# nnaisense/evotorch

Measured on NVIDIA H100. Metric: PGPE generations/sec at popsize=1Mxdim=10k (Rastrigin, fp32), higher is better.
Workload: dtype f32

## Files before the change

### evotorch_b200/_native.py

```python

from __future__ import annotations

import ctypes
import os
from ctypes import c_float, c_int, c_int64, c_size_t, c_uint64, c_void_p
from typing import Optional

import torch

_PKG = os.path.dirname(os.path.abspath(__file__))
LIB_PATH = os.path.join(_PKG, "lib", "libevok.so")

_P = c_void_p
_SIGNATURES = {
    "evok_abi_version": (c_int, []),
    "evok_launch_count": (c_uint64, []),
    "evok_error_string": (ctypes.c_char_p, [c_int]),
    "evok_sample_eval": (c_int, [c_int, _P, c_int64, _P, _P, c_int64, c_int64, c_int64, c_int, c_uint64, c_uint64, _P, _P, _P]),
    "evok_eval": (c_int, [c_int, _P, c_int64, c_int64, c_int64, _P, _P]),
    "evok_rank_workspace_bytes": (c_size_t, [c_int64]),
    "evok_rank": (c_int, [c_int, _P, c_int64, c_int, _P, _P, _P, c_size_t, _P]),
    "evok_argsort": (c_int, [_P, c_int64, c_int, _P, _P, c_size_t, _P]),
    "evok_sample_batched": (c_int, [_P, c_int64, c_int64, _P, c_int64, _P, c_int64, c_int64, c_int64, c_int64, c_int, c_uint64, c_uint64, _P]),
    "evok_rank_batched": (c_int, [c_int, _P, c_int64, c_int64, c_int, _P, _P, c_size_t, _P]),
# ... 2 lines not shown
    "evok_grad_batched_workspace_bytes": (c_size_t, [c_int64, c_int64, c_int64]),
    "evok_grad_batched": (c_int, [c_int, _P, c_int64, c_int64, _P, _P, c_int64, _P, c_int64, c_int64, c_int64, c_int64, c_float, c_float, _P, _P, _P,
                                  c_size_t, _P]),
    "evok_clipup_batched": (c_int, [_P, c_int64, c_int64, _P, _P, _P, _P, _P, _P]),
    "evok_sigma_update_batched": (c_int, [_P, _P, c_int64, c_int64, _P, c_int, _P, _P, _P, _P]),
    "evok_rank_table": (c_int, [_P, c_int64, c_int, _P, _P, _P, c_size_t, _P]),
    "evok_cholesky_workspace_bytes": (c_size_t, [c_int64]),
    "evok_cholesky": (c_int, [_P, c_int64, c_int64, _P, c_int64, _P, c_size_t, _P]),
    "evok_cmaes_row_weights": (c_int, [_P, _P, c_int64, c_int64, c_int64, c_int, _P, _P, _P]),
    "evok_cmaes_vector_update": (c_int, [_P, _P, c_int64, _P, _P, _P, _P, _P, c_int64, _P, c_int, _P, _P, _P]),
    "evok_sample_eval_sq": (c_int, [c_int, _P, c_int64, _P, _P, c_int64, c_int64, c_int64, c_uint64, c_uint64, _P, _P, _P, _P]),
    "evok_sepcma_workspace_bytes": (c_size_t, [c_int64, c_int64]),
    "evok_sepcma_moments": (c_int, [_P, _P, c_int, c_int64, c_int64, c_int64, c_uint64, c_uint64, _P, _P, _P, _P, _P, c_size_t, _P]),
    "evok_sepcma_update": (c_int, [_P, _P, _P, c_int64, _P, _P, _P, _P, _P, _P, _P, _P, _P, _P, c_int64, _P, c_int, c_int64, c_float, c_float, _P,
                                   _P]),
    "evok_weights_adjust": (c_int, [_P, c_int64, c_int, _P]),
    "evok_elite_mask": (c_int, [_P, c_int64, c_int64, _P, _P, c_size_t, _P]),
    "evok_grad_workspace_bytes": (c_size_t, [c_int64, c_int64]),
    "evok_grad": (c_int, [c_int, _P, c_int64, _P, _P, _P, c_int64, c_int64, c_float, c_float, _P, _P, _P, c_size_t, _P]),
    "evok_grad_regen": (c_int, [c_int, _P, _P, _P, c_int64, c_int64, c_int64, c_uint64, c_uint64, _P, c_float, c_float, _P, _P, _P,
                                c_size_t, _P]),
    "evok_grad_hybrid": (c_int, [c_int, _P, c_int64, _P, _P, _P, c_int64, c_int64, c_int64, c_uint64, c_uint64, _P, c_int, c_float, c_float, _P,
                                 _P, _P, c_size_t, _P]),
    "evok_grad_auto_split": (c_int, [c_int64]),
    "evok_grad_power_limit_mw": (c_int64, [c_int]),
    "evok_clipup_step": (c_int, [_P, c_int64, _P, c_float, c_float, c_float, _P, _P, _P]),
    "evok_adam_step": (c_int, [_P, c_int64, _P, _P, c_int64, c_float, c_float, c_float, c_float, _P, _P, _P]),
    "evok_sgd_step": (c_int, [_P, c_int64, _P, c_int, c_float, c_float, _P, _P, _P]),
    "evok_axpy": (c_int, [_P, c_int64, c_float, _P, _P]),
    "evok_sigma_update": (c_int, [_P, _P, c_int64, c_float, c_int, _P, c_float, _P, c_float, _P, c_float, _P]),
    "evok_cem_finalize": (c_int, [_P, _P, _P, c_int64, c_int64, _P, _P, _P]),
    "evok_mlp_parameter_length": (c_int64, [c_int, _P]),
    "evok_mlp_forward": (c_int, [_P, c_int64, _P, c_int64, _P, c_int64, c_int64, c_int, _P, _P, _P]),
    "evok_mlp_forward_prep": (c_int, [_P, c_int64, _P, c_int64, _P, c_int64, c_int64, c_int, _P, _P, _P, _P, _P, c_float, c_float, c_float, _P, _P,
                                      c_size_t, _P]),
    "evok_mlp_forward_shared_supported": (c_int, [c_int, _P]),
    "evok_mlp_forward_shared_workspace_bytes": (c_size_t, [c_int64, c_int64, c_int, _P]),
    "evok_mlp_forward_shared": (c_int, [_P, c_int64, c_int64, _P, c_int64, c_int64, c_int, _P, _P, _P, _P, c_size_t, _P]),
    "evok_gemm_gather_rows": (c_int, [_P, c_int64, c_int64, c_int64, c_int64, _P, c_int64, c_int64, c_int64, c_int64, c_int, _P, c_int64, _P]),
    "evok_gemm_gather_rows_workspace_bytes": (c_size_t, [c_int64, c_int64]),
    "evok_gemm_gather_rows_ws": (c_int, [_P, c_int64, c_int64, c_int64, c_int64, _P, c_int64, c_int64, c_int64, c_int64, c_int, _P, c_int64, c_int, _P, c_size_t, _P]),
    "evok_gemm_workspace_bytes": (c_size_t, [c_int64, c_int64, c_int64]),
    "evok_gemm_nt": (c_int, [_P, c_int64, _P, c_int64, c_int64, c_int64, c_int64, _P, c_int64, _P, c_int64, _P, _P, _P, c_size_t, _P]),
    "evok_gemm_nt_affine": (c_int, [_P, c_int64, _P, c_int64, c_int64, c_int64, c_int64, _P, c_int64, _P, _P, c_int64, _P, _P, c_size_t, _P]),
    "evok_transpose_pair": (c_int, [_P, c_int64, c_int64, c_int64, _P, _P, _P, c_int64, _P]),
    "evok_transpose_scale": (c_int, [_P, c_int64, c_int64, c_int64, _P, _P, c_int64, _P]),
# ... 102 lines not shown
```

### evotorch_b200/csrc/evok_common.cuh

```cuda
#pragma once

#include <cuda_runtime.h>
#include <stdint.h>

#include "../../include/evok.h"

#define EVOK_CHECK_LAUNCH_N(n)                       \
  do {                                               \
    cudaError_t e__ = cudaPeekAtLastError();         \
    if (e__ != cudaSuccess) return (int)e__;         \
    evok::count_launches(n);                         \
  } while (0)
#define EVOK_CHECK_LAUNCH() EVOK_CHECK_LAUNCH_N(1)

namespace evok {

extern unsigned long long g_launch_count;
inline void count_launches(int n) { __atomic_fetch_add(&g_launch_count, (unsigned long long)n, __ATOMIC_RELAXED); }

constexpr int kWarp = 32;
constexpr int kNumSMs = 132;

struct PeerSink {
  void* data[EVOK_MAX_PEERS];
// ... 78 lines not shown
}

__device__ __forceinline__ void box_muller(uint32_t a, uint32_t b, float& z0, float& z1) {
  const float u1 = fmaf((float)a, 2.3283064365386963e-10f, 1.1641532182693481e-10f);
  const float th = fmaf((float)b, 1.4629180792671596e-09f, 7.314590396335798e-10f);
  const float r = sqrt_approx(lg2_approx(u1) * -1.3862943611198906f);
  float s, c;
  __sincosf(th, &s, &c);
  z0 = r * c;
  z1 = r * s;
}

__device__ __forceinline__ void normals4(const PhiloxKey& key, uint32_t stream_word, uint64_t unit, uint32_t q, float z[4]) {
  U4 c;
  c.x = q;
  c.y = (uint32_t)unit;
  c.z = (uint32_t)(unit >> 32);
  c.w = stream_word;
  const U4 r = philox4x32_10(c, key);
  box_muller(r.x, r.y, z[0], z[1]);
  box_muller(r.z, r.w, z[2], z[3]);
}

__device__ __forceinline__ float warp_sum(float v) {
#pragma unroll
  for (int o = 16; o > 0; o >>= 1) v += __shfl_xor_sync(0xffffffffu, v, o);
  return v;
}
__device__ __forceinline__ double warp_sum(double v) {
#pragma unroll
  for (int o = 16; o > 0; o >>= 1) v += __shfl_xor_sync(0xffffffffu, v, o);
  return v;
}

template <typename T>
__device__ __forceinline__ T block_sum(T v, T* smem ) {
  const int lane = threadIdx.x & 31, wid = threadIdx.x >> 5, nw = (blockDim.x + 31) >> 5;
  v = warp_sum(v);
  __syncthreads();
  if (lane == 0) smem[wid] = v;
  __syncthreads();
  if (wid == 0) {
    T t = lane < nw ? smem[lane] : T(0);
    t = warp_sum(t);
    if (lane == 0) smem[32] = t;
  }
// ... 91 lines not shown
```

### evotorch_b200/csrc/evok_grad.cu

```cuda
#include <dlfcn.h>

#include <atomic>
#include <cstdlib>

#include "evok_common.cuh"

#ifndef EVOK_GRAD_TMA_DEFAULT
#define EVOK_GRAD_TMA_DEFAULT 1
#endif

namespace evok {

#ifndef EVOK_GRAD_UNROLL
#define EVOK_GRAD_UNROLL 4
#endif
#ifndef EVOK_GRAD_MINB
#define EVOK_GRAD_MINB 4
#endif
#ifndef EVOK_GRAD_CTAS_PER_SM
#define EVOK_GRAD_CTAS_PER_SM 4
#endif
constexpr int kGradThreads = 256;
constexpr int kGradUnroll = EVOK_GRAD_UNROLL;
constexpr int kMaxResidentCtas = kNumSMs * 8;
// ... 231 lines not shown
static int launch_finalize(const float* partial, int n_chunks, int64_t D, float scale_mu, float scale_sigma, float* out_mu, float* out_sigma,
                           const GradPush* push, cudaStream_t st) {
  const unsigned grid = (unsigned)((D + 255) / 256);
  if (push) grad_finalize_push_kernel<<<grid, 256, 0, st>>>(partial, n_chunks, D, scale_mu, scale_sigma, push->sink, push->epoch, push->done);
  else grad_finalize_kernel<<<grid, 256, 0, st>>>(partial, n_chunks, D, scale_mu, scale_sigma, out_mu, out_sigma);
  EVOK_CHECK_LAUNCH();
  return 0;
}

#ifndef EVOK_GRAD_TMA_ROWS
#define EVOK_GRAD_TMA_ROWS 4
#endif
#ifndef EVOK_GRAD_TMA_STAGES
#define EVOK_GRAD_TMA_STAGES 4
#endif
#ifndef EVOK_GRAD_TMA_CTAS_PER_SM
#define EVOK_GRAD_TMA_CTAS_PER_SM 3
#endif
constexpr int kTmaRows = EVOK_GRAD_TMA_ROWS;
constexpr int kTmaStages = EVOK_GRAD_TMA_STAGES;
constexpr int kTmaCols = 1024;
constexpr int kTmaConsumers = 256;
constexpr int kTmaThreads = kTmaConsumers + 32;
constexpr size_t kTmaSmemBytes = (size_t)kTmaStages * kTmaRows * kTmaCols * sizeof(float) + 2 * kTmaStages * sizeof(uint64_t) + 128;

__device__ __forceinline__ uint32_t smem_u32(const void* p) { return (uint32_t)__cvta_generic_to_shared(p); }
__device__ __forceinline__ void mbar_init(uint64_t* bar, uint32_t count) {
  asm volatile("mbarrier.init.shared::cta.b64 [%0], %1;" ::"r"(smem_u32(bar)), "r"(count) : "memory");
}
__device__ __forceinline__ void mbar_expect_tx(uint64_t* bar, uint32_t bytes) {
  asm volatile("mbarrier.arrive.expect_tx.shared::cta.b64 _, [%0], %1;" ::"r"(smem_u32(bar)), "r"(bytes) : "memory");
}
__device__ __forceinline__ void mbar_arrive(uint64_t* bar) {
  asm volatile("mbarrier.arrive.shared::cta.b64 _, [%0];" ::"r"(smem_u32(bar)) : "memory");
}
__device__ __forceinline__ void mbar_wait(uint64_t* bar, uint32_t parity) {
  asm volatile(
      "{\n"
      ".reg .pred P1;\n"
      "LAB_WAIT:\n"
      "mbarrier.try_wait.parity.shared::cta.b64 P1, [%0], %1;\n"
      "@P1 bra DONE;\n"
      "bra LAB_WAIT;\n"
      "DONE:\n"
      "}" ::"r"(smem_u32(bar)), "r"(parity) : "memory");
}
__device__ __forceinline__ void bulk_load(void* dst_smem, const void* src_gmem, uint32_t bytes, uint64_t* bar) {
  asm volatile("cp.async.bulk.shared::cluster.global.mbarrier::complete_tx::bytes [%0], [%1], %2, [%3];" ::"r"(smem_u32(dst_smem)),
               "l"(src_gmem), "r"(bytes), "r"(smem_u32(bar))
               : "memory");
}

constexpr int kSplitPeriod = 16;
__device__ __forceinline__ uint32_t rebuilt_mask(int split) {
  uint32_t m = 0;
#pragma unroll
  for (int k = 0; k < kSplitPeriod; ++k)
    if ((k + 1) * split / kSplitPeriod > k * split / kSplitPeriod) m |= 1u << k;
  return m;
}
__device__ __forceinline__ bool group_rebuilt(uint32_t mask, int64_t g) { return (mask >> ((int)g & (kSplitPeriod - 1))) & 1u; }

template <bool SYM>
__global__ void __launch_bounds__(kTmaThreads, EVOK_GRAD_TMA_CTAS_PER_SM)
    grad_partial_tma_kernel(int form, const float* __restrict__ X, int64_t ldx, const float* __restrict__ w, const float* __restrict__ mu,
                            const float* __restrict__ sigma, int64_t n_units, int64_t D, int64_t units_per_chunk, int split, uint64_t unit0,
                            const __grid_constant__ PhiloxKey key, const uint32_t* __restrict__ stream_off, float* __restrict__ partial) {
  extern __shared__ __align__(128) unsigned char smem_raw[];
  float* tiles = reinterpret_cast<float*>(smem_raw);
  uint64_t* full = reinterpret_cast<uint64_t*>(smem_raw + (size_t)kTmaStages * kTmaRows * kTmaCols * sizeof(float));
  uint64_t* empty = full + kTmaStages;

  const int tid = threadIdx.x, warp = tid >> 5, lane = tid & 31;
  const int64_t col0 = (int64_t)blockIdx.x * kTmaCols;
  const int64_t width = min((int64_t)kTmaCols, D - col0);
  const int64_t r_begin = (int64_t)blockIdx.y * units_per_chunk;
  const int64_t r_end = min(n_units, r_begin + units_per_chunk);
  const int64_t n_rows = r_end - r_begin;
  const int64_t n_groups = (n_rows + kTmaRows - 1) / kTmaRows;
  const int64_t row_stride = (SYM ? 2 : 1) * ldx;
  const uint32_t mask = rebuilt_mask(split);

  if (tid == 0) {
    for (int s = 0; s < kTmaStages; ++s) {
      mbar_init(&full[s], 1);
      mbar_init(&empty[s], kTmaConsumers / 32);
    }
    asm volatile("fence.mbarrier_init.release.cluster;" ::: "memory");
  }
  __syncthreads();

  if (warp == kTmaConsumers / 32) {
    if (lane == 0) {
      const uint32_t row_bytes = (uint32_t)(width * sizeof(float));
      int64_t t = 0;
      for (int64_t g = 0; g < n_groups; ++g) {
        if (group_rebuilt(mask, g)) continue;
        const int s = (int)(t % kTmaStages);
        const uint32_t use = (uint32_t)(t / kTmaStages);
        ++t;
        if (use > 0) mbar_wait(&empty[s], (use - 1) & 1);
        const int64_t r0 = r_begin + g * kTmaRows;
        const int rows = (int)min((int64_t)kTmaRows, r_end - r0);
        mbar_expect_tx(&full[s], rows * row_bytes);
        float* dst = tiles + (size_t)s * kTmaRows * kTmaCols;
        for (int i = 0; i < rows; ++i) bulk_load(dst + (size_t)i * kTmaCols, X + (r0 + i) * row_stride + col0, row_bytes, &full[s]);
      }
    }
    return;
  }

  const int64_t col = col0 + (int64_t)tid * 4;
  const bool active = col < D;
  const uint32_t sw = key.stream_lo + (stream_off ? __ldg(stream_off) : 0u);
  const int frm = SYM ? EVOK_GRAD_SYMMETRIC : form;
  float m[4], sg[4], c1[4], c0[4];
#pragma unroll
  for (int c = 0; c < 4; ++c) {
    sg[c] = active ? __ldg(sigma + col + c) : 1.0f;
    m[c] = active ? __ldg(mu + col + c) : 0.0f;
    if (frm == EVOK_GRAD_EXP) {
      c1[c] = __fdiv_rn(1.0f, sg[c] * sg[c]);
      c0[c] = 1.0f;
    } else if (frm == EVOK_GRAD_MOMENTS) {
      c1[c] = 1.0f;
      c0[c] = 0.0f;
    } else {
      c1[c] = __fdiv_rn(1.0f, sg[c]);
      c0[c] = sg[c];
    }
  }
  float s1[4] = {0.f, 0.f, 0.f, 0.f}, s2[4] = {0.f, 0.f, 0.f, 0.f};

  int64_t t = 0;
  for (int64_t g = 0; g < n_groups; ++g) {
    const int64_t r0 = r_begin + g * kTmaRows;
    const int rows = (int)min((int64_t)kTmaRows, r_end - r0);
    float a[kTmaRows], b[kTmaRows];
    bool need[kTmaRows];
#pragma unroll
    for (int i = 0; i < kTmaRows; ++i) {
      a[i] = b[i] = 0.0f;
      if (i < rows) {
        if (SYM) {
          const float wp = __ldg(w + 2 * (r0 + i)), wm = __ldg(w + 2 * (r0 + i) + 1);
          a[i] = 0.5f * (wp - wm);
          b[i] = 0.5f * (wp + wm);
        } else {
          a[i] = b[i] = __ldg(w + r0 + i);
        }
      }
      need[i] = a[i] != 0.0f || b[i] != 0.0f;
    }
    if (group_rebuilt(mask, g)) {
      if (active) {
        float x[kTmaRows][4];
#pragma unroll
        for (int i = 0; i < kTmaRows; ++i) {
          float z[4];
          normals4(key, sw, unit0 + (uint64_t)(r0 + i), (uint32_t)(col >> 2), z);
#pragma unroll
          for (int c = 0; c < 4; ++c) x[i][c] = fmaf(sg[c], z[c], m[c]);
        }
#pragma unroll
        for (int i = 0; i < kTmaRows; ++i) {
          if (need[i]) {
#pragma unroll
            for (int c = 0; c < 4; ++c) {
              const float e = x[i][c] - m[c];
              s1[c] = fmaf(a[i], e, s1[c]);
              s2[c] = fmaf(b[i], fmaf(e * e, c1[c], -c0[c]), s2[c]);
            }
          }
        }
      }
      continue;
    }
    const int s = (int)(t % kTmaStages);
    const uint32_t use = (uint32_t)(t / kTmaStages);
    ++t;
    mbar_wait(&full[s], use & 1);
    const float4* tile = reinterpret_cast<const float4*>(tiles + (size_t)s * kTmaRows * kTmaCols) + tid;
    if (active) {
      float4 v4[kTmaRows];
#pragma unroll
      for (int i = 0; i < kTmaRows; ++i) v4[i] = tile[(size_t)i * (kTmaCols / 4)];
#pragma unroll
      for (int i = 0; i < kTmaRows; ++i) {
        if (need[i]) {
          const float4 v = v4[i];
          const float x[4] = {v.x, v.y, v.z, v.w};
#pragma unroll
          for (int c = 0; c < 4; ++c) {
            const float e = x[c] - m[c];
            s1[c] = fmaf(a[i], e, s1[c]);
            s2[c] = fmaf(b[i], fmaf(e * e, c1[c], -c0[c]), s2[c]);
          }
        }
      }
    }
    __syncwarp();
    if (lane == 0) mbar_arrive(&empty[s]);
  }
  if (active) {
    float* p1 = partial + ((int64_t)blockIdx.y * 2 + 0) * D + col;
    float* p2 = partial + ((int64_t)blockIdx.y * 2 + 1) * D + col;
#pragma unroll
    for (int c = 0; c < 4; ++c) {
      p1[c] = s1[c];
      p2[c] = s2[c];
    }
  }
}

struct GradPlan {
  int vec, tx, n_coltiles, n_chunks;
  int64_t units_per_chunk;
};

static GradPlan plan_grad(int64_t n_units, int64_t D, bool vec_ok) {
  GradPlan p;
  p.vec = vec_ok ? 4 : 1;
  const int64_t col_threads = (D + p.vec - 1) / p.vec;
  p.tx = 32;
  while (p.tx < kGradThreads && p.tx < col_threads) p.tx <<= 1;
  p.n_coltiles = (int)((col_threads + p.tx - 1) / p.tx);
// ... 41 lines not shown
    cudaGetLastError();
    return -1;
  }
  void* nvml = dlopen("libnvidia-ml.so.1", RTLD_NOW | RTLD_LOCAL);
  if (!nvml) return -1;
  using init_t = int (*)();
  using by_bus_t = int (*)(const char*, void**);
  using limit_t = int (*)(void*, unsigned int*);
  const auto init = reinterpret_cast<init_t>(dlsym(nvml, "nvmlInit_v2"));
  const auto shutdown = reinterpret_cast<init_t>(dlsym(nvml, "nvmlShutdown"));
  const auto by_bus = reinterpret_cast<by_bus_t>(dlsym(nvml, "nvmlDeviceGetHandleByPciBusId_v2"));
  const auto limit = reinterpret_cast<limit_t>(dlsym(nvml, "nvmlDeviceGetEnforcedPowerLimit"));
  int64_t mw = -1;
  if (init && shutdown && by_bus && limit && init() == 0) {
    void* handle = nullptr;
    unsigned int v = 0;
    if (by_bus(bus_id, &handle) == 0 && limit(handle, &v) == 0) mw = v;
    shutdown();
  }
  dlclose(nvml);
  return mw;
}

static int device_auto_split() {
  constexpr int kMaxDevices = 64;
  static std::atomic<int> resolved[kMaxDevices];
  int device = 0;
  if (cudaGetDevice(&device) != cudaSuccess || device < 0 || device >= kMaxDevices) {
    cudaGetLastError();
    return kAutoSplitCapped;
  }
  int s = resolved[device].load(std::memory_order_relaxed);
  if (s == 0) {
    s = auto_split_for_power(enforced_power_limit_mw(device)) + 1;
    resolved[device].store(s, std::memory_order_relaxed);
  }
  return s - 1;
}

static int grad_impl(int form, const float* X, int64_t ldx, const float* w, const float* mu, const float* sigma, int64_t row0, int64_t n_rows,
                     int64_t D, bool regen, uint64_t seed, uint64_t stream_id, const uint32_t* stream_off, float scale_mu, float scale_sigma, float* out_mu,
                     float* out_sigma, void* ws, size_t ws_bytes, void* stream, const GradPush* push = nullptr, int split = 0) {
  if (!w || !mu || !sigma || !ws || (!regen && !X) || (!push && (!out_mu || !out_sigma))) return EVOK_E_NULLPTR;
  if (form < EVOK_GRAD_SEPARABLE || form > EVOK_GRAD_MOMENTS) return EVOK_E_BADENUM;
  if (n_rows < 0 || D <= 0 || row0 < 0 || (!regen && ldx < D) || split < -1 || split > kSplitPeriod) return EVOK_E_BADSIZE;
  const bool sym = form == EVOK_GRAD_SYMMETRIC;
  if (sym && ((n_rows & 1) || (row0 & 1))) return EVOK_E_ODDROWS;
  if (ws_bytes < evok_grad_workspace_bytes(n_rows, D)) return EVOK_E_WORKSPACE;
  cudaStream_t st = (cudaStream_t)stream;
  const int64_t n_units = sym ? n_rows / 2 : n_rows;
  const bool vec_ok = regen ? true : ((D % 4 == 0) && (ldx % 4 == 0) && aligned16(X));
  const uint64_t unit0 = (uint64_t)(sym ? row0 / 2 : row0);
  GradPlan p = plan_grad(n_units, D, vec_ok);
  float* partial = (float*)ws;
  if (n_units == 0 && push) return launch_finalize(partial, 0, D, scale_mu, scale_sigma, nullptr, nullptr, push, st);
  if (n_units == 0) {
    cudaMemsetAsync(out_mu, 0, (size_t)D * 4, st);
    cudaMemsetAsync(out_sigma, 0, (size_t)D * 4, st);
    return 0;
  }
  const char* tma_env = getenv("EVOK_GRAD_TMA");
  const int use_tma = tma_env ? atoi(tma_env) : EVOK_GRAD_TMA_DEFAULT;
  if (use_tma && !regen && vec_ok && form != EVOK_GRAD_MOMENTS && D >= 512 && n_units >= 4096) {
    const int n_coltiles = (int)((D + kTmaCols - 1) / kTmaCols);
    int64_t chunks = (int64_t)kNumSMs * EVOK_GRAD_TMA_CTAS_PER_SM / n_coltiles;
    if (chunks < 1) chunks = 1;
    if (chunks > 65535) chunks = 65535;
    const int64_t upc = (n_units + chunks - 1) / chunks;
    const int n_chunks = (int)((n_units + upc - 1) / upc);
    dim3 grid(n_coltiles, n_chunks);
    const int rebuilt = split < 0 ? device_auto_split() : split;
    const PhiloxKey key = make_philox_key(seed, stream_id);
    auto kernel = sym ? grad_partial_tma_kernel<true> : grad_partial_tma_kernel<false>;
    cudaFuncSetAttribute(kernel, cudaFuncAttributeMaxDynamicSharedMemorySize, (int)kTmaSmemBytes);
    kernel<<<grid, kTmaThreads, kTmaSmemBytes, st>>>(form, X, ldx, w, mu, sigma, n_units, D, upc, rebuilt, unit0, key, stream_off, partial);
    EVOK_CHECK_LAUNCH();
    return launch_finalize(partial, n_chunks, D, scale_mu, scale_sigma, out_mu, out_sigma, push, st);
  }
  if (regen) {
    if (sym) launch_partial<4, true, true>(p, form, X, ldx, w, mu, sigma, n_units, D, unit0, seed, stream_id, stream_off, partial, st);
    else launch_partial<4, false, true>(p, form, X, ldx, w, mu, sigma, n_units, D, unit0, seed, stream_id, stream_off, partial, st);
  } else if (vec_ok) {
    if (sym) launch_partial<4, true, false>(p, form, X, ldx, w, mu, sigma, n_units, D, unit0, seed, stream_id, stream_off, partial, st);
    else launch_partial<4, false, false>(p, form, X, ldx, w, mu, sigma, n_units, D, unit0, seed, stream_id, stream_off, partial, st);
  } else {
    if (sym) launch_partial<1, true, false>(p, form, X, ldx, w, mu, sigma, n_units, D, unit0, seed, stream_id, stream_off, partial, st);
    else launch_partial<1, false, false>(p, form, X, ldx, w, mu, sigma, n_units, D, unit0, seed, stream_id, stream_off, partial, st);
  }
  EVOK_CHECK_LAUNCH();
  return launch_finalize(partial, p.n_chunks, D, scale_mu, scale_sigma, out_mu, out_sigma, push, st);
}

}

using namespace evok;

extern "C" EVOK_API size_t evok_grad_workspace_bytes(int64_t n_rows, int64_t D) {
  (void)n_rows;
  if (D <= 0) return 256;
  return ((size_t)kMaxResidentCtas * 1024 + 2 * (size_t)D + 64) * sizeof(float);
}

extern "C" EVOK_API int evok_grad(int form, const float* X, int64_t ldx, const float* w, const float* mu, const float* sigma, int64_t n_rows,
                         int64_t D, float scale_mu, float scale_sigma, float* out_mu, float* out_sigma, void* ws, size_t ws_bytes,
                         void* stream) {
  return grad_impl(form, X, ldx, w, mu, sigma, 0, n_rows, D, false, 0, 0, nullptr, scale_mu, scale_sigma, out_mu, out_sigma, ws, ws_bytes, stream);
}

extern "C" EVOK_API int evok_grad_regen(int form, const float* w, const float* mu, const float* sigma, int64_t row0, int64_t n_rows, int64_t D,
                               uint64_t seed, uint64_t stream_id, const uint32_t* stream_offset_dev, float scale_mu, float scale_sigma,
                               float* out_mu, float* out_sigma, void* ws, size_t ws_bytes, void* stream) {
  return grad_impl(form, nullptr, 0, w, mu, sigma, row0, n_rows, D, true, seed, stream_id, stream_offset_dev, scale_mu, scale_sigma, out_mu, out_sigma, ws,
                   ws_bytes, stream);
}

extern "C" EVOK_API int evok_grad_hybrid(int form, const float* X, int64_t ldx, const float* w, const float* mu, const float* sigma, int64_t row0,
                                         int64_t n_rows, int64_t D, uint64_t seed, uint64_t stream_id, const uint32_t* stream_offset_dev, int split,
                                         float scale_mu, float scale_sigma, float* out_mu, float* out_sigma, void* ws, size_t ws_bytes, void* stream) {
  return grad_impl(form, X, ldx, w, mu, sigma, row0, n_rows, D, false, seed, stream_id, stream_offset_dev, scale_mu, scale_sigma, out_mu, out_sigma, ws,
                   ws_bytes, stream, nullptr, split);
}

extern "C" EVOK_API int evok_grad_auto_split(int64_t power_limit_mw) { return auto_split_for_power(power_limit_mw); }

extern "C" EVOK_API int64_t evok_grad_power_limit_mw(int device) { return enforced_power_limit_mw(device); }

extern "C" EVOK_API size_t evok_sepcma_workspace_bytes(int64_t n_rows, int64_t D) {
  return evok_grad_workspace_bytes(n_rows, D) + (size_t)kMaxResidentCtas * sizeof(float);
}

extern "C" EVOK_API int evok_sepcma_moments(const float* aw, const float* q, int active, int64_t row0, int64_t n_rows, int64_t D, uint64_t seed,
                                            uint64_t stream_id, const uint32_t* stream_offset_dev, float* local, float* S2, float* wsum, void* ws,
                                            size_t ws_bytes, void* stream) {
  if (!aw || (active && !q) || !local || !S2 || !wsum || !ws) return EVOK_E_NULLPTR;
  if (n_rows <= 0 || D <= 0 || row0 < 0) return EVOK_E_BADSIZE;
  if (ws_bytes < evok_sepcma_workspace_bytes(n_rows, D)) return EVOK_E_WORKSPACE;
  cudaStream_t st = (cudaStream_t)stream;
  const GradPlan p = plan_grad(n_rows, D, true);
  float* partial = (float*)ws;
  const SepWeights sep{q, active, partial + evok_grad_workspace_bytes(n_rows, D) / sizeof(float)};
  launch_partial<4, false, true, true>(p, EVOK_GRAD_MOMENTS, nullptr, 0, aw, nullptr, nullptr, n_rows, D, (uint64_t)row0, seed, stream_id,
                                       stream_offset_dev, partial, st, 1, nullptr, &sep);
  EVOK_CHECK_LAUNCH();
  grad_finalize_kernel<true><<<(unsigned)((D + 255) / 256), 256, 0, st>>>(partial, p.n_chunks, D, 1.0f, 1.0f, local, S2, 0, sep.wsum_partial, wsum);
// ... 77 lines not shown
```

### evotorch_b200/ops.py

```python

from __future__ import annotations

import ctypes
import math
from typing import Optional

import torch

from . import _native as nat
from .tools.readonlytensor import as_plain_tensor

OBJ_NONE, OBJ_SPHERE, OBJ_RASTRIGIN, OBJ_ACKLEY = 0, 1, 2, 3
OBJECTIVE_IDS = {"sphere": OBJ_SPHERE, "rastrigin": OBJ_RASTRIGIN, "ackley": OBJ_ACKLEY}
RANK_IDS = {"centered": 0, "linear": 1, "nes": 2, "normalized": 3, "raw": 4}
GRAD_SEPARABLE, GRAD_SYMMETRIC, GRAD_EXP, GRAD_MOMENTS = 0, 1, 2, 3
NAN = float("nan")


_timers: Optional[dict] = None


def enable_timers() -> None:
    global _timers
    _timers = {}
# ... 317 lines not shown
    with _timed("grad"):
        rc = nat.lib().evok_grad(form, X.data_ptr(), X.stride(0), w.data_ptr(), mu.data_ptr(), sigma.data_ptr(), n, D, scale_mu,
                                 scale_sigma, out_mu.data_ptr(), out_sigma.data_ptr(), ws.data_ptr(), ws.numel(), nat.stream_of(X))
    nat.check(rc, "evok_grad")
    return out_mu, out_sigma


def grad_regen(form: int, w: torch.Tensor, mu: torch.Tensor, sigma: torch.Tensor, *, seed: int, stream_id: int, row0: int,
               scale_mu: float, scale_sigma: float, out_mu: Optional[torch.Tensor] = None,
               out_sigma: Optional[torch.Tensor] = None, stream_offset: Optional[torch.Tensor] = None) -> tuple:
    n, D = w.numel(), mu.numel()
    _vec(w, "weights"); _vec(mu, "mu"); _vec(sigma, "sigma", D)
    out_mu, out_sigma = _out_pair(mu, out_mu, out_sigma)
    ws = nat.workspace(mu.device, nat.lib().evok_grad_workspace_bytes(n, D), "grad")
    with _timed("grad_regen"):
        rc = nat.lib().evok_grad_regen(form, w.data_ptr(), mu.data_ptr(), sigma.data_ptr(), row0, n, D, seed, stream_id,
                                       _offset_ptr(stream_offset), scale_mu, scale_sigma, out_mu.data_ptr(), out_sigma.data_ptr(),
                                       ws.data_ptr(), ws.numel(), nat.stream_of(mu))
    nat.check(rc, "evok_grad_regen")
    return out_mu, out_sigma


GRAD_SPLIT_PERIOD = 16


def grad_hybrid(form: int, X: torch.Tensor, w: torch.Tensor, mu: torch.Tensor, sigma: torch.Tensor, *, seed: int, stream_id: int, row0: int,
                scale_mu: float, scale_sigma: float, split: int = -1, out_mu: Optional[torch.Tensor] = None,
                out_sigma: Optional[torch.Tensor] = None, stream_offset: Optional[torch.Tensor] = None) -> tuple:
    _mat(X, "samples")
    n, D = X.shape
    _vec(w, "weights", n); _vec(mu, "mu", D); _vec(sigma, "sigma", D)
    if not -1 <= split <= GRAD_SPLIT_PERIOD:
        raise ValueError(f"split: expected -1 .. {GRAD_SPLIT_PERIOD}, got {split}")
    out_mu, out_sigma = _out_pair(mu, out_mu, out_sigma)
    ws = nat.workspace(X.device, nat.lib().evok_grad_workspace_bytes(n, D), "grad")
    with _timed("grad_hybrid"):
        rc = nat.lib().evok_grad_hybrid(form, X.data_ptr(), X.stride(0), w.data_ptr(), mu.data_ptr(), sigma.data_ptr(), row0, n, D,
                                        seed, stream_id, _offset_ptr(stream_offset), int(split), scale_mu, scale_sigma,
                                        out_mu.data_ptr(), out_sigma.data_ptr(), ws.data_ptr(), ws.numel(), nat.stream_of(X))
    nat.check(rc, "evok_grad_hybrid")
    return out_mu, out_sigma


def clipup_step(g: torch.Tensor, velocity: torch.Tensor, stepsize: float, momentum: float, max_speed: float,
                step_out: Optional[torch.Tensor] = None, mu: Optional[torch.Tensor] = None) -> None:
    D = g.numel()
    _vec(g, "g"); _vec(velocity, "velocity", D)
    with _timed("mu_step"):
        rc = nat.lib().evok_clipup_step(g.data_ptr(), D, velocity.data_ptr(), stepsize, momentum, max_speed, nat.ptr(step_out),
                                        nat.ptr(mu), nat.stream_of(g))
    nat.check(rc, "evok_clipup_step")


def adam_step(g: torch.Tensor, m: torch.Tensor, v: torch.Tensor, t: int, lr: float, beta1: float, beta2: float, eps: float,
              step_out: Optional[torch.Tensor] = None, mu: Optional[torch.Tensor] = None) -> None:
    D = g.numel()
    _vec(g, "g"); _vec(m, "m", D); _vec(v, "v", D)
    rc = nat.lib().evok_adam_step(g.data_ptr(), D, m.data_ptr(), v.data_ptr(), t, lr, beta1, beta2, eps, nat.ptr(step_out), nat.ptr(mu),
                                  nat.stream_of(g))
    nat.check(rc, "evok_adam_step")


# ... 301 lines not shown
```

### include/evok.h

```cpp
#ifndef EVOK_H_
#define EVOK_H_

#include <stddef.h>
#include <stdint.h>

#ifdef __cplusplus
extern "C" {
#endif

#define EVOK_ABI_VERSION 1

#if defined(__GNUC__)
#define EVOK_API __attribute__((visibility("default")))
#else
#define EVOK_API
#endif

#define EVOK_E_NULLPTR (-1)
#define EVOK_E_BADSIZE (-2)
#define EVOK_E_BADENUM (-3)
#define EVOK_E_WORKSPACE (-4)
#define EVOK_E_ODDROWS (-5)
#define EVOK_E_ALIGN (-6)

#define EVOK_MAX_PEERS 16

#define EVOK_OBJ_NONE 0
#define EVOK_OBJ_SPHERE 1
#define EVOK_OBJ_RASTRIGIN 2
#define EVOK_OBJ_ACKLEY 3
#define EVOK_OBJ_COUNT 4

#define EVOK_RANK_CENTERED 0
#define EVOK_RANK_LINEAR 1
#define EVOK_RANK_NES 2
#define EVOK_RANK_NORMALIZED 3
#define EVOK_RANK_RAW 4

#define EVOK_GRAD_SEPARABLE 0
#define EVOK_GRAD_SYMMETRIC 1
#define EVOK_GRAD_EXP 2
#define EVOK_GRAD_MOMENTS 3

int evok_abi_version(void);
uint64_t evok_launch_count(void);
const char* evok_error_string(int code);

int evok_sample_eval(int objective, float* X, int64_t ldx, const float* mu, const float* sigma, int64_t row0,
                     int64_t n_rows, int64_t D, int symmetric, uint64_t seed, uint64_t stream_id,
                     const uint32_t* stream_offset_dev, float* f, void* stream);

int evok_eval(int objective, const float* X, int64_t ldx, int64_t n_rows, int64_t D, float* f, void* stream);

size_t evok_rank_workspace_bytes(int64_t N);
int evok_rank(int method, const float* f, int64_t N, int higher_is_better, float* w, int64_t* perm, void* ws,
              size_t ws_bytes, void* stream);

int evok_argsort(const float* keys, int64_t N, int descending, int64_t* perm, void* ws, size_t ws_bytes,
                 void* stream);

int evok_rank_table(const float* keys, int64_t N, int descending, const float* table, float* out, void* ws, size_t ws_bytes, void* stream);

int evok_weights_adjust(float* w, int64_t N, int mode, void* stream);

int evok_elite_mask(const float* w, int64_t N, int64_t num_elites, float* mask, void* ws, size_t ws_bytes,
                    void* stream);

size_t evok_grad_workspace_bytes(int64_t n_rows, int64_t D);
int evok_grad(int form, const float* X, int64_t ldx, const float* w, const float* mu, const float* sigma,
              int64_t n_rows, int64_t D, float scale_mu, float scale_sigma, float* out_mu, float* out_sigma,
              void* ws, size_t ws_bytes, void* stream);

int evok_grad_regen(int form, const float* w, const float* mu, const float* sigma, int64_t row0, int64_t n_rows,
                    int64_t D, uint64_t seed, uint64_t stream_id, const uint32_t* stream_offset_dev, float scale_mu,
                    float scale_sigma, float* out_mu, float* out_sigma, void* ws, size_t ws_bytes, void* stream);

int evok_grad_hybrid(int form, const float* X, int64_t ldx, const float* w, const float* mu, const float* sigma, int64_t row0,
                     int64_t n_rows, int64_t D, uint64_t seed, uint64_t stream_id, const uint32_t* stream_offset_dev, int split,
                     float scale_mu, float scale_sigma, float* out_mu, float* out_sigma, void* ws, size_t ws_bytes, void* stream);

int evok_grad_auto_split(int64_t power_limit_mw);

int64_t evok_grad_power_limit_mw(int device);

int evok_clipup_step(const float* g, int64_t D, float* velocity, float stepsize, float momentum, float max_speed,
                     float* step_out, float* mu, void* stream);
int evok_adam_step(const float* g, int64_t D, float* m, float* v, int64_t t, float lr, float beta1, float beta2,
                   float eps, float* step_out, float* mu, void* stream);
int evok_sgd_step(const float* g, int64_t D, float* buf, int first_step, float lr, float momentum, float* step_out,
                  float* mu, void* stream);
int evok_axpy(const float* g, int64_t D, float lr, float* mu, void* stream);

int evok_sigma_update(float* sigma, const float* g, int64_t D, float lr, int exp_form, const float* lb_vec,
                      float lb, const float* ub_vec, float ub, const float* mc_vec, float mc, void* stream);

int evok_cem_finalize(const float* s1, const float* s2, const float* sigma, int64_t D, int64_t num_elites,
                      float* grad_mu, float* grad_sigma, void* stream);

#define EVOK_ACT_NONE 0
#define EVOK_ACT_TANH 1
#define EVOK_ACT_RELU 2
#define EVOK_ACT_SIGMOID 3
// ... 91 lines not shown
```

Before: 49.38.

## Add runtime-adaptive rebuild scheduling and hoisted Philox invariants to hybrid grad kernel

Adds a runtime schedule mode in which the TMA producer decides per group whether to load a tile or let consumers regenerate it, driven by a consumer 'want' flag raised when a full barrier is not yet ready. It also hoists the first Philox rounds that depend only on the high unit word and column into precomputed invariants, so regenerated rows compute fewer rounds. The default path still uses the static schedule, but the Philox invariant shortcut applies to every rebuilt group. The runtime mode adds shared-memory spin polling and volatile flags, and there is optional clock64 profiling behind a macro.

```diff
diff --git a/evotorch_b200/_native.py b/evotorch_b200/_native.py
--- a/evotorch_b200/_native.py
+++ b/evotorch_b200/_native.py
@@ -48,6 +48,8 @@
                                 c_size_t, _P]),
     "evok_grad_hybrid": (c_int, [c_int, _P, c_int64, _P, _P, _P, c_int64, c_int64, c_int64, c_uint64, c_uint64, _P, c_int, c_float, c_float, _P,
                                  _P, _P, c_size_t, _P]),
+    "evok_grad_hybrid_sched": (c_int, [c_int, _P, c_int64, _P, _P, _P, c_int64, c_int64, c_int64, c_uint64, c_uint64, _P, c_int, c_int, c_float,
+                                       c_float, _P, _P, _P, c_size_t, _P]),
     "evok_grad_auto_split": (c_int, [c_int64]),
     "evok_grad_power_limit_mw": (c_int64, [c_int]),
     "evok_clipup_step": (c_int, [_P, c_int64, _P, c_float, c_float, c_float, _P, _P, _P]),
diff --git a/evotorch_b200/csrc/evok_common.cuh b/evotorch_b200/csrc/evok_common.cuh
--- a/evotorch_b200/csrc/evok_common.cuh
+++ b/evotorch_b200/csrc/evok_common.cuh
@@ -124,6 +124,47 @@
   box_muller(r.z, r.w, z[2], z[3]);
 }
 
+struct PhiloxUnitInvariants {
+  uint32_t x1, w1, y2, hi3, lo3;
+};
+
+__device__ __forceinline__ PhiloxUnitInvariants philox_unit_invariants(const PhiloxKey& key, uint32_t stream_word, uint32_t unit_hi, uint32_t q) {
+  constexpr uint32_t M0 = 0xD2511F53u, M1 = 0xCD9E8D57u;
+  PhiloxUnitInvariants v;
+  v.x1 = __umulhi(M1, unit_hi) ^ key.k0[0];
+  const uint32_t y1 = M1 * unit_hi, z1 = __umulhi(M0, q) ^ stream_word ^ key.k1[0];
+  v.w1 = (M0 * q) ^ key.k1[1];
+  const uint32_t x2 = __umulhi(M1, z1) ^ y1 ^ key.k0[1];
+  v.y2 = (M1 * z1) ^ key.k0[2];
+  v.hi3 = __umulhi(M0, x2) ^ key.k1[2];
+  v.lo3 = M0 * x2;
+  return v;
+}
+
+__device__ __forceinline__ void normals4_unit(const PhiloxKey& key, const PhiloxUnitInvariants& v, uint32_t unit_lo, float z[4]) {
+  constexpr uint32_t M0 = 0xD2511F53u, M1 = 0xCD9E8D57u;
+  const uint32_t x1 = v.x1 ^ unit_lo;
+  const uint32_t z2 = __umulhi(M0, x1) ^ v.w1, w2 = M0 * x1;
+  U4 c;
+  c.x = __umulhi(M1, z2) ^ v.y2;
+  c.y = M1 * z2;
+  c.z = v.hi3 ^ w2;
+  c.w = v.lo3;
+#pragma unroll
+  for (int r = 3; r < EVOK_PHILOX_ROUNDS; ++r) {
+    const uint32_t hi0 = __umulhi(M0, c.x), lo0 = M0 * c.x;
+    const uint32_t hi1 = __umulhi(M1, c.z), lo1 = M1 * c.z;
+    U4 n;
+    n.x = hi1 ^ c.y ^ key.k0[r];
+    n.y = lo1;
+    n.z = hi0 ^ c.w ^ key.k1[r];
+    n.w = lo0;
+    c = n;
+  }
+  box_muller(c.x, c.y, z[0], z[1]);
+  box_muller(c.z, c.w, z[2], z[3]);
+}
+
 __device__ __forceinline__ float warp_sum(float v) {
 #pragma unroll
   for (int o = 16; o > 0; o >>= 1) v += __shfl_xor_sync(0xffffffffu, v, o);
diff --git a/evotorch_b200/csrc/evok_grad.cu b/evotorch_b200/csrc/evok_grad.cu
--- a/evotorch_b200/csrc/evok_grad.cu
+++ b/evotorch_b200/csrc/evok_grad.cu
@@ -277,7 +277,8 @@
 constexpr int kTmaCols = 1024;
 constexpr int kTmaConsumers = 256;
 constexpr int kTmaThreads = kTmaConsumers + 32;
-constexpr size_t kTmaSmemBytes = (size_t)kTmaStages * kTmaRows * kTmaCols * sizeof(float) + 2 * kTmaStages * sizeof(uint64_t) + 128;
+constexpr size_t kTmaSmemBytes =
+    (size_t)kTmaStages * kTmaRows * kTmaCols * sizeof(float) + 2 * kTmaStages * sizeof(uint64_t) + (kTmaStages + 2) * sizeof(uint32_t) + 128;
 
 __device__ __forceinline__ uint32_t smem_u32(const void* p) { return (uint32_t)__cvta_generic_to_shared(p); }
 __device__ __forceinline__ void mbar_init(uint64_t* bar, uint32_t count) {
@@ -300,6 +301,19 @@
       "DONE:\n"
       "}" ::"r"(smem_u32(bar)), "r"(parity) : "memory");
 }
+__device__ __forceinline__ bool mbar_test(uint64_t* bar, uint32_t parity) {
+  uint32_t done;
+  asm volatile(
+      "{\n"
+      ".reg .pred P1;\n"
+      "mbarrier.test_wait.parity.shared::cta.b64 P1, [%1], %2;\n"
+      "selp.u32 %0, 1, 0, P1;\n"
+      "}"
+      : "=r"(done)
+      : "r"(smem_u32(bar)), "r"(parity)
+      : "memory");
+  return done != 0;
+}
 __device__ __forceinline__ void bulk_load(void* dst_smem, const void* src_gmem, uint32_t bytes, uint64_t* bar) {
   asm volatile("cp.async.bulk.shared::cluster.global.mbarrier::complete_tx::bytes [%0], [%1], %2, [%3];" ::"r"(smem_u32(dst_smem)),
                "l"(src_gmem), "r"(bytes), "r"(smem_u32(bar))
@@ -316,15 +330,38 @@
 }
 __device__ __forceinline__ bool group_rebuilt(uint32_t mask, int64_t g) { return (mask >> ((int)g & (kSplitPeriod - 1))) & 1u; }
 
+struct GroupSchedule {
+  uint32_t tag[kTmaStages];
+  uint32_t decided;
+  uint32_t want;
+};
+
+#ifdef EVOK_GRAD_PROFILE
+enum { kProfFullWait, kProfEmptyWait, kProfRebuild, kProfConsume, kProfRebuiltGroups, kProfGroups, kProfCtaCycles, kProfSlots };
+constexpr int kProfMaxCtas = kMaxResidentCtas;
+__device__ unsigned long long g_grad_prof[kProfMaxCtas][kProfSlots];
+#define EVOK_PROF_CLOCK(v) const long long v = clock64()
+#define EVOK_PROF_ADD(slot, v) (prof[slot] += (unsigned)(v))
+#else
+#define EVOK_PROF_CLOCK(v)
+#define EVOK_PROF_ADD(slot, v)
+#endif
+
 template <bool SYM>
 __global__ void __launch_bounds__(kTmaThreads, EVOK_GRAD_TMA_CTAS_PER_SM)
     grad_partial_tma_kernel(int form, const float* __restrict__ X, int64_t ldx, const float* __restrict__ w, const float* __restrict__ mu,
-                            const float* __restrict__ sigma, int64_t n_units, int64_t D, int64_t units_per_chunk, int split, uint64_t unit0,
-                            const __grid_constant__ PhiloxKey key, const uint32_t* __restrict__ stream_off, float* __restrict__ partial) {
+                            const float* __restrict__ sigma, int64_t n_units, int64_t D, int64_t units_per_chunk, int split, int sched,
+                            uint64_t unit0, const __grid_constant__ PhiloxKey key, const uint32_t* __restrict__ stream_off,
+                            float* __restrict__ partial) {
   extern __shared__ __align__(128) unsigned char smem_raw[];
   float* tiles = reinterpret_cast<float*>(smem_raw);
   uint64_t* full = reinterpret_cast<uint64_t*>(smem_raw + (size_t)kTmaStages * kTmaRows * kTmaCols * sizeof(float));
   uint64_t* empty = full + kTmaStages;
+  volatile GroupSchedule* gs = reinterpret_cast<volatile GroupSchedule*>(empty + kTmaStages);
+#ifdef EVOK_GRAD_PROFILE
+  unsigned prof[kProfSlots] = {};
+  EVOK_PROF_CLOCK(prof_t0);
+#endif
 
   const int tid = threadIdx.x, warp = tid >> 5, lane = tid & 31;
   const int64_t col0 = (int64_t)blockIdx.x * kTmaCols;
@@ -340,7 +377,10 @@
     for (int s = 0; s < kTmaStages; ++s) {
       mbar_init(&full[s], 1);
       mbar_init(&empty[s], kTmaConsumers / 32);
-    }
+      gs->tag[s] = 0xFFFFFFFFu;
+    }
+    gs->decided = 0;
+    gs->want = 0;
     asm volatile("fence.mbarrier_init.release.cluster;" ::: "memory");
   }
   __syncthreads();
@@ -349,19 +389,36 @@
     if (lane == 0) {
       const uint32_t row_bytes = (uint32_t)(width * sizeof(float));
       int64_t t = 0;
+      int64_t held = -1;
       for (int64_t g = 0; g < n_groups; ++g) {
         if (group_rebuilt(mask, g)) continue;
         const int s = (int)(t % kTmaStages);
         const uint32_t use = (uint32_t)(t / kTmaStages);
-        ++t;
-        if (use > 0) mbar_wait(&empty[s], (use - 1) & 1);
-        const int64_t r0 = r_begin + g * kTmaRows;
-        const int rows = (int)min((int64_t)kTmaRows, r_end - r0);
-        mbar_expect_tx(&full[s], rows * row_bytes);
-        float* dst = tiles + (size_t)s * kTmaRows * kTmaCols;
-        for (int i = 0; i < rows; ++i) bulk_load(dst + (size_t)i * kTmaCols, X + (r0 + i) * row_stride + col0, row_bytes, &full[s]);
-      }
-    }
+        if (sched != EVOK_GRAD_SCHED_REBUILD_ALL && held != t) {
+          EVOK_PROF_CLOCK(w0);
+          if (use > 0) mbar_wait(&empty[s], (use - 1) & 1);
+          EVOK_PROF_ADD(kProfEmptyWait, clock64() - w0);
+          held = t;
+        }
+        const bool rebuild = sched == EVOK_GRAD_SCHED_REBUILD_ALL || (sched == EVOK_GRAD_SCHED_RUNTIME && gs->want);
+        if (rebuild) {
+          gs->want = 0;
+        } else {
+          const int64_t r0 = r_begin + g * kTmaRows;
+          const int rows = (int)min((int64_t)kTmaRows, r_end - r0);
+          mbar_expect_tx(&full[s], rows * row_bytes);
+          float* dst = tiles + (size_t)s * kTmaRows * kTmaCols;
+          for (int i = 0; i < rows; ++i) bulk_load(dst + (size_t)i * kTmaCols, X + (r0 + i) * row_stride + col0, row_bytes, &full[s]);
+          gs->tag[s] = (uint32_t)g;
+          ++t;
+        }
+        __threadfence_block();
+        gs->decided = (uint32_t)(g + 1);
+      }
+    }
+#ifdef EVOK_GRAD_PROFILE
+    if (lane == 0) atomicAdd(&g_grad_prof[blockIdx.y * gridDim.x + blockIdx.x][kProfEmptyWait], (unsigned long long)prof[kProfEmptyWait]);
+#endif
     return;
   }
 
@@ -386,6 +443,9 @@
     }
   }
   float s1[4] = {0.f, 0.f, 0.f, 0.f}, s2[4] = {0.f, 0.f, 0.f, 0.f};
+  const uint32_t q = (uint32_t)(col >> 2);
+  uint32_t inv_hi = (uint32_t)((unit0 + (uint64_t)r_begin) >> 32);
+  PhiloxUnitInvariants inv = philox_unit_invariants(key, sw, inv_hi, q);
 
   int64_t t = 0;
   for (int64_t g = 0; g < n_groups; ++g) {
@@ -407,15 +467,41 @@
       }
       need[i] = a[i] != 0.0f || b[i] != 0.0f;
     }
-    if (group_rebuilt(mask, g)) {
+    bool rebuilt = group_rebuilt(mask, g);
+    if (!rebuilt && sched != EVOK_GRAD_SCHED_STATIC) {
+      EVOK_PROF_CLOCK(d0);
+      while (gs->decided <= (uint32_t)g) {
+      }
+      EVOK_PROF_ADD(kProfFullWait, clock64() - d0);
+      __threadfence_block();
+      rebuilt = gs->tag[t % kTmaStages] != (uint32_t)g;
+    }
+    if (rebuilt) {
+      EVOK_PROF_CLOCK(b0);
       if (active) {
+        const uint64_t u0 = unit0 + (uint64_t)r0;
+        const uint32_t hi = (uint32_t)(u0 >> 32);
         float x[kTmaRows][4];
-#pragma unroll
-        for (int i = 0; i < kTmaRows; ++i) {
-          float z[4];
-          normals4(key, sw, unit0 + (uint64_t)(r0 + i), (uint32_t)(col >> 2), z);
-#pragma unroll
-          for (int c = 0; c < 4; ++c) x[i][c] = fmaf(sg[c], z[c], m[c]);
+        if (hi == (uint32_t)((u0 + kTmaRows - 1) >> 32)) {
+          if (hi != inv_hi) {
+            inv_hi = hi;
+            inv = philox_unit_invariants(key, sw, hi, q);
+          }
+#pragma unroll
+          for (int i = 0; i < kTmaRows; ++i) {
+            float z[4];
+            normals4_unit(key, inv, (uint32_t)u0 + (uint32_t)i, z);
+#pragma unroll
+            for (int c = 0; c < 4; ++c) x[i][c] = fmaf(sg[c], z[c], m[c]);
+          }
+        } else {
+#pragma unroll
+          for (int i = 0; i < kTmaRows; ++i) {
+            float z[4];
+            normals4(key, sw, u0 + (uint64_t)i, q, z);
+#pragma unroll
+            for (int c = 0; c < 4; ++c) x[i][c] = fmaf(sg[c], z[c], m[c]);
+          }
         }
 #pragma unroll
         for (int i = 0; i < kTmaRows; ++i) {
@@ -429,12 +515,20 @@
           }
         }
       }
+      EVOK_PROF_ADD(kProfRebuild, clock64() - b0);
+      EVOK_PROF_ADD(kProfRebuiltGroups, 1);
       continue;
     }
     const int s = (int)(t % kTmaStages);
     const uint32_t use = (uint32_t)(t / kTmaStages);
     ++t;
-    mbar_wait(&full[s], use & 1);
+    if (!mbar_test(&full[s], use & 1)) {
+      EVOK_PROF_CLOCK(f0);
+      gs->want = 1;
+      mbar_wait(&full[s], use & 1);
+      EVOK_PROF_ADD(kProfFullWait, clock64() - f0);
+    }
+    EVOK_PROF_CLOCK(c0_);
     const float4* tile = reinterpret_cast<const float4*>(tiles + (size_t)s * kTmaRows * kTmaCols) + tid;
     if (active) {
       float4 v4[kTmaRows];
@@ -456,7 +550,21 @@
     }
     __syncwarp();
     if (lane == 0) mbar_arrive(&empty[s]);
-  }
+    EVOK_PROF_ADD(kProfConsume, clock64() - c0_);
+  }
+#ifdef EVOK_GRAD_PROFILE
+  if (lane == 0) {
+    unsigned long long* dst = g_grad_prof[blockIdx.y * gridDim.x + blockIdx.x];
+    atomicAdd(&dst[kProfFullWait], (unsigned long long)prof[kProfFullWait]);
+    atomicAdd(&dst[kProfRebuild], (unsigned long long)prof[kProfRebuild]);
+    atomicAdd(&dst[kProfConsume], (unsigned long long)prof[kProfConsume]);
+    if (warp == 0) {
+      atomicAdd(&dst[kProfRebuiltGroups], (unsigned long long)prof[kProfRebuiltGroups]);
+      atomicAdd(&dst[kProfGroups], (unsigned long long)n_groups);
+      atomicAdd(&dst[kProfCtaCycles], (unsigned long long)(clock64() - prof_t0));
+    }
+  }
+#endif
   if (active) {
     float* p1 = partial + ((int64_t)blockIdx.y * 2 + 0) * D + col;
     float* p2 = partial + ((int64_t)blockIdx.y * 2 + 1) * D + col;
@@ -544,27 +652,29 @@
   return mw;
 }
 
-static int device_auto_split() {
+static int64_t device_power_limit_mw() {
   constexpr int kMaxDevices = 64;
-  static std::atomic<int> resolved[kMaxDevices];
+  static std::atomic<int64_t> resolved[kMaxDevices];
   int device = 0;
   if (cudaGetDevice(&device) != cudaSuccess || device < 0 || device >= kMaxDevices) {
     cudaGetLastError();
-    return kAutoSplitCapped;
-  }
-  int s = resolved[device].load(std::memory_order_relaxed);
-  if (s == 0) {
-    s = auto_split_for_power(enforced_power_limit_mw(device)) + 1;
-    resolved[device].store(s, std::memory_order_relaxed);
-  }
-  return s - 1;
+    return -1;
+  }
+  int64_t v = resolved[device].load(std::memory_order_relaxed);
+  if (v == 0) {
+    v = enforced_power_limit_mw(device) + 2;
+    resolved[device].store(v, std::memory_order_relaxed);
+  }
+  return v - 2;
 }
 
 static int grad_impl(int form, const float* X, int64_t ldx, const float* w, const float* mu, const float* sigma, int64_t row0, int64_t n_rows,
                      int64_t D, bool regen, uint64_t seed, uint64_t stream_id, const uint32_t* stream_off, float scale_mu, float scale_sigma, float* out_mu,
-                     float* out_sigma, void* ws, size_t ws_bytes, void* stream, const GradPush* push = nullptr, int split = 0) {
+                     float* out_sigma, void* ws, size_t ws_bytes, void* stream, const GradPush* push = nullptr, int split = 0,
+                     int sched = EVOK_GRAD_SCHED_STATIC) {
   if (!w || !mu || !sigma || !ws || (!regen && !X) || (!push && (!out_mu || !out_sigma))) return EVOK_E_NULLPTR;
   if (form < EVOK_GRAD_SEPARABLE || form > EVOK_GRAD_MOMENTS) return EVOK_E_BADENUM;
+  if (sched < EVOK_GRAD_SCHED_STATIC || sched > EVOK_GRAD_SCHED_REBUILD_ALL) return EVOK_E_BADENUM;
   if (n_rows < 0 || D <= 0 || row0 < 0 || (!regen && ldx < D) || split < -1 || split > kSplitPeriod) return EVOK_E_BADSIZE;
   const bool sym = form == EVOK_GRAD_SYMMETRIC;
   if (sym && ((n_rows & 1) || (row0 & 1))) return EVOK_E_ODDROWS;
@@ -591,11 +701,12 @@
     const int64_t upc = (n_units + chunks - 1) / chunks;
     const int n_chunks = (int)((n_units + upc - 1) / upc);
     dim3 grid(n_coltiles, n_chunks);
-    const int rebuilt = split < 0 ? device_auto_split() : split;
+    const int rebuilt = split < 0 ? auto_split_for_power(device_power_limit_mw()) : split;
     const PhiloxKey key = make_philox_key(seed, stream_id);
     auto kernel = sym ? grad_partial_tma_kernel<true> : grad_partial_tma_kernel<false>;
     cudaFuncSetAttribute(kernel, cudaFuncAttributeMaxDynamicSharedMemorySize, (int)kTmaSmemBytes);
-    kernel<<<grid, kTmaThreads, kTmaSmemBytes, st>>>(form, X, ldx, w, mu, sigma, n_units, D, upc, rebuilt, unit0, key, stream_off, partial);
+    kernel<<<grid, kTmaThreads, kTmaSmemBytes, st>>>(form, X, ldx, w, mu, sigma, n_units, D, upc, rebuilt, sched, unit0, key, stream_off,
+                                                     partial);
     EVOK_CHECK_LAUNCH();
     return launch_finalize(partial, n_chunks, D, scale_mu, scale_sigma, out_mu, out_sigma, push, st);
   }
@@ -640,8 +751,27 @@
                                          int64_t n_rows, int64_t D, uint64_t seed, uint64_t stream_id, const uint32_t* stream_offset_dev, int split,
                                          float scale_mu, float scale_sigma, float* out_mu, float* out_sigma, void* ws, size_t ws_bytes, void* stream) {
   return grad_impl(form, X, ldx, w, mu, sigma, row0, n_rows, D, false, seed, stream_id, stream_offset_dev, scale_mu, scale_sigma, out_mu, out_sigma, ws,
-                   ws_bytes, stream, nullptr, split);
-}
+                   ws_bytes, stream, nullptr, split, EVOK_GRAD_SCHED_STATIC);
+}
+
+extern "C" EVOK_API int evok_grad_hybrid_sched(int form, const float* X, int64_t ldx, const float* w, const float* mu, const float* sigma,
+                                               int64_t row0, int64_t n_rows, int64_t D, uint64_t seed, uint64_t stream_id,
+                                               const uint32_t* stream_offset_dev, int split, int sched, float scale_mu, float scale_sigma,
+                                               float* out_mu, float* out_sigma, void* ws, size_t ws_bytes, void* stream) {
+  return grad_impl(form, X, ldx, w, mu, sigma, row0, n_rows, D, false, seed, stream_id, stream_offset_dev, scale_mu, scale_sigma, out_mu, out_sigma, ws,
+                   ws_bytes, stream, nullptr, split, sched);
+}
+
+#ifdef EVOK_GRAD_PROFILE
+extern "C" EVOK_API int evok_grad_profile_read(unsigned long long* host, int max_ctas) {
+  const int n = max_ctas < kProfMaxCtas ? max_ctas : kProfMaxCtas;
+  cudaDeviceSynchronize();
+  if (cudaMemcpyFromSymbol(host, g_grad_prof, (size_t)n * kProfSlots * sizeof(unsigned long long)) != cudaSuccess) return -1;
+  static unsigned long long zeros[kProfMaxCtas][kProfSlots];
+  if (cudaMemcpyToSymbol(g_grad_prof, zeros, sizeof(zeros)) != cudaSuccess) return -1;
+  return kProfSlots;
+}
+#endif
 
 extern "C" EVOK_API int evok_grad_auto_split(int64_t power_limit_mw) { return auto_split_for_power(power_limit_mw); }
 
diff --git a/evotorch_b200/ops.py b/evotorch_b200/ops.py
--- a/evotorch_b200/ops.py
+++ b/evotorch_b200/ops.py
@@ -363,22 +363,29 @@
 
 
 GRAD_SPLIT_PERIOD = 16
+GRAD_SCHED_STATIC, GRAD_SCHED_RUNTIME, GRAD_SCHED_REBUILD_ALL = 0, 1, 2
 
 
 def grad_hybrid(form: int, X: torch.Tensor, w: torch.Tensor, mu: torch.Tensor, sigma: torch.Tensor, *, seed: int, stream_id: int, row0: int,
-                scale_mu: float, scale_sigma: float, split: int = -1, out_mu: Optional[torch.Tensor] = None,
+                scale_mu: float, scale_sigma: float, split: int = -1, sched: Optional[int] = None, out_mu: Optional[torch.Tensor] = None,
                 out_sigma: Optional[torch.Tensor] = None, stream_offset: Optional[torch.Tensor] = None) -> tuple:
     _mat(X, "samples")
     n, D = X.shape
     _vec(w, "weights", n); _vec(mu, "mu", D); _vec(sigma, "sigma", D)
     if not -1 <= split <= GRAD_SPLIT_PERIOD:
         raise ValueError(f"split: expected -1 .. {GRAD_SPLIT_PERIOD}, got {split}")
+    if sched is not None and sched not in (GRAD_SCHED_STATIC, GRAD_SCHED_RUNTIME, GRAD_SCHED_REBUILD_ALL):
+        raise ValueError(f"sched: expected one of GRAD_SCHED_STATIC, GRAD_SCHED_RUNTIME, GRAD_SCHED_REBUILD_ALL, got {sched}")
     out_mu, out_sigma = _out_pair(mu, out_mu, out_sigma)
     ws = nat.workspace(X.device, nat.lib().evok_grad_workspace_bytes(n, D), "grad")
+    args = (form, X.data_ptr(), X.stride(0), w.data_ptr(), mu.data_ptr(), sigma.data_ptr(), row0, n, D, seed, stream_id,
+            _offset_ptr(stream_offset), int(split))
+    tail = (scale_mu, scale_sigma, out_mu.data_ptr(), out_sigma.data_ptr(), ws.data_ptr(), ws.numel(), nat.stream_of(X))
     with _timed("grad_hybrid"):
-        rc = nat.lib().evok_grad_hybrid(form, X.data_ptr(), X.stride(0), w.data_ptr(), mu.data_ptr(), sigma.data_ptr(), row0, n, D,
-                                        seed, stream_id, _offset_ptr(stream_offset), int(split), scale_mu, scale_sigma,
-                                        out_mu.data_ptr(), out_sigma.data_ptr(), ws.data_ptr(), ws.numel(), nat.stream_of(X))
+        if sched is None:
+            rc = nat.lib().evok_grad_hybrid(*args, *tail)
+        else:
+            rc = nat.lib().evok_grad_hybrid_sched(*args, int(sched), *tail)
     nat.check(rc, "evok_grad_hybrid")
     return out_mu, out_sigma
 
diff --git a/include/evok.h b/include/evok.h
--- a/include/evok.h
+++ b/include/evok.h
@@ -42,6 +42,10 @@
 #define EVOK_GRAD_EXP 2
 #define EVOK_GRAD_MOMENTS 3
 
+#define EVOK_GRAD_SCHED_STATIC 0
+#define EVOK_GRAD_SCHED_RUNTIME 1
+#define EVOK_GRAD_SCHED_REBUILD_ALL 2
+
 int evok_abi_version(void);
 uint64_t evok_launch_count(void);
 const char* evok_error_string(int code);
@@ -78,6 +82,11 @@
 int evok_grad_hybrid(int form, const float* X, int64_t ldx, const float* w, const float* mu, const float* sigma, int64_t row0,
                      int64_t n_rows, int64_t D, uint64_t seed, uint64_t stream_id, const uint32_t* stream_offset_dev, int split,
                      float scale_mu, float scale_sigma, float* out_mu, float* out_sigma, void* ws, size_t ws_bytes, void* stream);
+
+int evok_grad_hybrid_sched(int form, const float* X, int64_t ldx, const float* w, const float* mu, const float* sigma, int64_t row0,
+                           int64_t n_rows, int64_t D, uint64_t seed, uint64_t stream_id, const uint32_t* stream_offset_dev, int split,
+                           int sched, float scale_mu, float scale_sigma, float* out_mu, float* out_sigma, void* ws, size_t ws_bytes,
+                           void* stream);
 
 int evok_grad_auto_split(int64_t power_limit_mw);
 
```

Result: no change. 49.25 (median of 6 runs) (-0.3%).
